# iamgroot42/A-LINK

Measured on AMD Instinct MI355X. Metric: 112x112 face embeddings/sec (IR-ResNet-100 ArcFace, 512-d, L2-normalised), higher is better.
Workload: dtype bf16

## Files before the change

a-link_amd/csrc/alink_common.h:

```cpp
#pragma once
#include <hip/hip_runtime.h>
#include <stdint.h>
#include <stddef.h>
#include <string>

#include "../../include/alink_hip.h"
#include "conv_kernel.h"

namespace alink {

void set_error(const char* fmt, ...);
int  hip_fail(hipError_t e, const char* what, const char* file, int line);

#define ALINK_HIP(call)                                                          \
    do {                                                                         \
        hipError_t e__ = (call);                                                 \
        if (e__ != hipSuccess) return ::alink::hip_fail(e__, #call, __FILE__, __LINE__); \
    } while (0)

#define ALINK_REQUIRE(cond, code, ...)          \
    do {                                        \
        if (!(cond)) {                          \
            ::alink::set_error(__VA_ARGS__);    \
            return (code);                      \
// ... 50 lines not shown
    int post_relu;
    int fine;
    int stagger;
    int ablate;
    float acc_scale;
    float bias_scale;
    float res_scale;
    int nprod;
    void* stamps;
};

hipError_t launch_conv_igemm(int dtype, const ConvParams& p, hipStream_t stream);
double     conv_flops(const ConvParams& p);

struct StemParams {
    const void*  in;
    const void*  wgt;
    const float* bias;
    const float* alpha;
    void*        out;
    int N, H, W, C0, layout;
    float sub[3], mul;
    int flip;
    float acc_scale, bias_scale;
};
hipError_t launch_stem(int dtype, const StemParams& p, hipStream_t stream);

struct FcFinishParams {
    const float* slabs;
    const float* bias;
    float*       out;
    float*       norms;
    int S, M, E;
    float scale;
    int*  nonfinite;
};
hipError_t launch_fc_finish(const FcFinishParams& p, hipStream_t stream);
hipError_t launch_absmax_f16(const void* x, size_t n_elements, unsigned* out_bits, hipStream_t stream);
hipError_t launch_conv_split_finish(int dtype, const ConvParams& p, const float* slabs, int S, hipStream_t stream);

ConvKernel direct_variant(int ksz, int stride, int pad, int H, int W, int Cin, int Cout);
ConvKernel direct_variant_tiles(int ksz, int stride, int pad, int H, int W, int Cin, int Cout);
ConvKernel linear_variant_x2(int ksz, int stride, int pad, int H, int W, int Cin, int Cout);
hipError_t launch_conv(ConvKernel k, int dtype, const ConvParams& p, hipStream_t st);
hipError_t direct_set_attributes();
ConvKernel linear_variant(int ksz, int stride, int pad, int H, int W, int Cin, int Cout);
ConvKernel c64_variant(int ksz, int stride, int pad, int H, int W, int Cin, int Cout);
ConvKernel s2c64_variant(int ksz, int stride, int pad, int H, int W, int Cin, int Cout);
hipError_t launch_conv3x3_linear(ConvKernel k, int dtype, const ConvParams& p, hipStream_t st);
hipError_t launch_conv3x3_c64(int dtype, const ConvParams& p, hipStream_t st);
hipError_t launch_conv3x3_s2c64(int dtype, const ConvParams& p, hipStream_t st);
hipError_t c64_set_attributes();
hipError_t s2c64_set_attributes();
hipError_t linear_set_attributes();
hipError_t linear_check_contract();
bool       front_c64_applies(int dtype, int H, int W, int C0, int Cout);
hipError_t front_c64_set_attributes();
hipError_t launch_front_c64(int dtype, const ConvParams& conv1, const StemParams& stem, void* xs, bool slopes_le_1, hipStream_t st);
bool       unit_c64_applies(int dtype, const ConvParams& c1, const ConvParams& c2);
hipError_t unit_c64_set_attributes();
hipError_t launch_unit_c64(int dtype, const ConvParams& c1, const ConvParams& c2, hipStream_t st);
bool       conv3x3_lat_applies(int dtype, const ConvParams& p);
hipError_t launch_conv3x3_lat(int dtype, const ConvParams& p, hipStream_t stream);
bool       conv_gemm_lat_applies(int dtype, const ConvParams& p);
hipError_t launch_conv_gemm_lat(int dtype, const ConvParams& p, hipStream_t stream);

hipError_t launch_l2norm_bwd(int dtype, const float* g, const float* e, const float* norms, void* dz, int M, int E,
                             hipStream_t st);
hipError_t launch_zero_insert(int dtype, const void* in, void* out, int N, int H, int W, int Ho, int Wo, int C,
                              hipStream_t st);
hipError_t launch_stem_bwd(int dtype, const void* dy0, const void* y0, const float* w, const float* alpha, float* dpix,
                           int N, int H, int W, float mul, int nchw, hipStream_t st);

hipError_t launch_r50_grad_scale(const float* dfeat, int count, int HW, float* scale, hipStream_t st);
hipError_t launch_r50_avgpool_bwd(int dtype, const float* dfeat, const void* y, void* dz, const float* scale, int N, int HW, int C,
                                  hipStream_t st);
hipError_t launch_r50_relu_mask(int dtype, void* g, const void* y, long long count, hipStream_t st);
hipError_t launch_r50_scatter_mask(int dtype, const void* in, const void* y, void* out, int N, int H, int W, int Ho, int Wo, int C,
                                   hipStream_t st);
hipError_t launch_r50_maxpool_bwd(int dtype, const void* y0, const void* pooled, const void* g, void* d0, int N, int H, int W, int C,
                                  int Hp, int Wp, hipStream_t st);
hipError_t launch_r50_stem_bwd(int dtype, const void* d0, const void* wfrag, float* dpix, const float* scale, int N, int H, int W,
                               int Ho, int Wo, int pad_t, int pad_l, int flip, hipStream_t st);
int r50_stem_bwd_max_width();

uint16_t f32_to_bf16_rne(float f);
uint16_t f32_to_f16_rne(float f);

int init_kernels();

__device__ __forceinline__ float relu_keep_nan(float v) { return v < 0.f ? 0.f : v; }
__device__ __forceinline__ float max_keep_nan(float a, float b) { return (a < b || b != b) ? b : a; }

}
#include <map>
#include <string>
#include <vector>
namespace alink {
struct F32Net;
F32Net* f32net_build(const std::map<std::string, std::vector<float>>& raw, const alink_ir_cfg& cfg);
void    f32net_destroy(F32Net* n);
size_t  f32net_workspace_bytes(const F32Net* n, int N);
int     f32net_embed(const F32Net* n, const void* dev_in, int layout, int N, float* dev_out, void* ws, size_t ws_bytes,
                     hipStream_t st);

}
```

a-link_amd/csrc/backbone.hip:

```cpp
#include "alink_common.h"

#include <algorithm>
#include <cmath>
#include <cstdarg>
#include <cstdio>
#include <cstring>
#include <map>
#include <string>
#include <vector>

namespace alink {

static thread_local char g_err[1024] = "";
void set_error(const char* fmt, ...) {
    va_list ap;
    va_start(ap, fmt);
    vsnprintf(g_err, sizeof(g_err), fmt, ap);
    va_end(ap);
}
int hip_fail(hipError_t e, const char* what, const char* file, int line) {
    set_error("HIP error %d (%s) in `%s` at %s:%d", (int)e, hipGetErrorString(e), what, file, line);
    return ALINK_EHIP;
}

// ... 642 lines not shown
        const bool wide = (L.Cout % 128) == 0;
        nwg = wide ? ((M + 127) / 128) * (L.Cout / 128) : ((M + 255) / 256) * (L.Cout / 64);
        units = L.ksz * L.ksz * ncc; kpu = 1;
    } else {
        return 1;
    }
    if (nwg > 64) return 1;
    int best = 1;
    for (int S = 2; S <= 8; ++S)
        if (units % S == 0 && units / S * kpu >= 4 && nwg * S <= 512 && (size_t)S * M * L.Cout * 4 <= SPLIT_SLAB_BYTES) best = S;
    return best;
}

int g_sibling_aware = 1;
extern "C" void alink_debug_set_sibling_aware(int on) { g_sibling_aware = on != 0; }
int g_fine_max = 384;
extern "C" void alink_debug_set_fine_max(int n) { g_fine_max = n; }
static int fine_form(ConvKernel k, long long M, int Cout, int siblings = 1) {
    if (!traits(k).fine) return 0;
    const int sib = (g_sibling_aware && k != ConvKernel::Linear7) ? siblings : 1;
    return linear_grid(M, Cout, 128) * sib <= g_fine_max ? 1 : 0;
}
int g_ablate = 0;
int g_stop_after = 0;
extern "C" void alink_debug_set_stop_after(int n) { g_stop_after = n; }
int g_stagger = 0;
int g_shard_stagger = 0;
extern "C" void alink_debug_set_shard_stagger(int on) { g_shard_stagger = on; }

int g_fuse_unit = 1;
constexpr int FUSE_UNIT_MIN_N = 64;
extern "C" void alink_debug_set_fuse_unit(int mode) { g_fuse_unit = mode; }
extern "C" void alink_debug_set_stagger(int n) { g_stagger = n < 0 ? 0 : n; }
void* g_stamps = nullptr;
int g_prof_reps = 4;
extern "C" void alink_debug_set_profile_reps(int n) { g_prof_reps = n < 1 ? 1 : n; }
extern "C" void alink_debug_set_ablate(int a) { g_ablate = a; }
extern "C" void alink_debug_set_stamps(void* p) { g_stamps = p; }

static const ConvLayer* fusable_unit(const alink_backbone* bb, const ConvLayer& L, int N, int S, bool cache) {
    if (!g_fuse_unit || (g_fuse_unit == 1 && N < FUSE_UNIT_MIN_N) || cache || S != 1 || g_ablate || g_stamps) return nullptr;
    const int dt = bb->cfg.dtype;
    if (dt != ALINK_DT_BF16 && dt != ALINK_DT_F16) return nullptr;
    const size_t i = (size_t)(&L - bb->convs.data());
    if (L.role != 1 || i + 1 >= bb->convs.size()) return nullptr;
    const ConvLayer& L2 = bb->convs[i + 1];
    if (L2.role != 3 || L2.unit != L.unit || L2.Cin2 || L2.in_buf != L.out_buf || L2.resid_buf != L.in_buf) return nullptr;
    if (L.kernel != ConvKernel::Linear56 || L2.kernel != ConvKernel::Linear56 || L.stride != 1 || L2.stride != 1) return nullptr;
    if (L.Cin != 64 || L.Cout != 64 || L2.Cin != 64 || L2.Cout != 64 || L.Hin != 56 || L.Win != 56) return nullptr;
    if (plan_split(bb, L2, N) != 1) return nullptr;
    return &L2;
}

static int embed_impl(alink_backbone_t* bb, const void* dev_in, int layout, int N, float* dev_out,
                      void* ws, size_t ws_bytes, hipStream_t stream, float* ms, double* flops, int* kind,
                      int* n_launches, const GradLayout* cache = nullptr, int calib = 0, hipEvent_t front_done = nullptr) {
    ALINK_REQUIRE(bb && dev_in && dev_out && ws, ALINK_EINVAL, "NULL argument");
    ALINK_REQUIRE(bb->finalized, ALINK_ESTATE, "alink_embed before alink_backbone_finalize");
    ALINK_REQUIRE(N > 0, ALINK_EINVAL, "n_images must be positive");
    ALINK_REQUIRE(layout >= 0 && layout <= 2, ALINK_EINVAL, "unknown pixel layout %d", layout);
    const alink_ir_cfg& cfg = bb->cfg;
    ALINK_REQUIRE((long long)N * cfg.height * cfg.width * 64 * (cfg.dtype == ALINK_DT_F16X2 ? 2 : 1) < (1ll << 31), ALINK_EINVAL,
                  "batch of %d images exceeds the 2^31-element activation limit; split the batch", N);
    size_t off[7], total;
    ws_layout(bb, N, off, &total);
    if (cache) total = cache->total;
    ALINK_REQUIRE(ws_bytes >= total, ALINK_ENOMEM, "workspace too small: %zu < %zu", ws_bytes, total);
    ALINK_REQUIRE(((uintptr_t)ws & 255) == 0, ALINK_EINVAL, "workspace must be 256-byte aligned");
    char* base = (char*)ws;
    auto buf = [&](int id) -> void* { return base + off[id]; };

    const bool prof = ms != nullptr;
    const int reps = prof ? g_prof_reps : 1;
    const int cap = prof ? *n_launches : 0;
    int nl = 0;
    std::vector<hipEvent_t> ev;
    std::vector<int> split_pairs;
    auto mark = [&]() -> int {
        if (!prof) return ALINK_OK;
        hipEvent_t e;
        ALINK_HIP(hipEventCreate(&e));
        ALINK_HIP(hipEventRecord(e, stream));
        ev.push_back(e);
        return ALINK_OK;
    };
    auto note = [&](double f, int k) {
        if (prof && nl < cap) { flops[nl] = f; kind[nl] = k; }
        ++nl;
    };
    int rc;
    if ((rc = mark())) return rc;

    const bool x2 = cfg.dtype == ALINK_DT_F16X2;
    ALINK_REQUIRE(!calib || x2, ALINK_ESTATE, "only the split-precision mode is calibrated");
    ALINK_REQUIRE(!x2 || calib || bb->calibrated, ALINK_ESTATE, "split-precision backbone: alink_backbone_calibrate has not run");
    int bexp[5] = {0, 0, 0, 0, 0};
    auto settle = [&](int* e_io, const void* out, size_t n_elems, auto&& launch) -> int {
        int e = *e_io;
        for (int attempt = 0; attempt < 24; ++attempt) {
            const int rcl = launch(e);
            if (rcl) return rcl;
            if (!calib) break;
            unsigned bits = 0;
            ALINK_HIP(hipMemsetAsync(bb->d_absmax, 0, 4, stream));
            ALINK_HIP(launch_absmax_f16(out, n_elems, bb->d_absmax, stream));
            ALINK_HIP(hipMemcpyAsync(&bits, bb->d_absmax, 4, hipMemcpyDeviceToHost, stream));
// ... 38 lines not shown
    }

    int last_out = 0, n_done = 0;
    bool front_marked = false;
    bool skip_conv2 = false;
    for (ConvLayer& L : bb->convs) {
        if (skip_conv2) { skip_conv2 = false; continue; }
        if (g_stop_after && n_done++ >= g_stop_after) return ALINK_OK;
        if (front_done && !front_marked && L.stage >= 1) {
            ALINK_HIP(hipEventRecord(front_done, stream));
            front_marked = true;
        }
        ConvParams p{};
        p.in = buf(L.in_buf); p.wgt = L.d_w; p.bias = L.d_bias; p.alpha = L.d_alpha;
        p.resid = L.resid_buf >= 0 ? buf(L.resid_buf) : nullptr;
        p.out = buf(L.out_buf); p.zero = bb->d_zero;
        if (cache) {
            if (L.role == 1) p.out = base + cache->toff[L.unit];
            if (L.role == 3) p.in = base + cache->toff[L.unit];
        }
        p.N = N; p.H = L.Hin; p.W = L.Win; p.Cin = L.Cin; p.Cout = L.Cout; p.Ho = L.Hout; p.Wo = L.Wout;
        p.stride = L.stride; p.ksz = L.ksz; p.pad = L.pad; p.M = N * L.Hout * L.Wout;
        p.border_cls = L.border_cls ? 1 : 0; p.splitk = 1;
        p.ksteps_per_split = L.ksz * L.ksz * (L.Cin / 64) + L.Cin2 / 64;
        if (L.Cin2) { p.in2 = buf(L.in2_buf); p.Cin2 = L.Cin2; p.in2_compact = (front && &L == &bb->convs[1]) ? 1 : 0; }
        p.ablate = g_ablate;
        p.stagger = g_stagger;
        p.nprod = (x2 && !calib) ? bb->products : 0;
        p.fine = fine_form(L.kernel, p.M, L.Cout, bb->siblings);
        int S = plan_split(bb, L, N);
        if (S > 1) {
            ConvParams probe = p;
            probe.splitk = 1;
            if (traits(L.kernel).split == SplitUnit::Chunk ? conv3x3_lat_applies(cfg.dtype, probe) : conv_gemm_lat_applies(cfg.dtype, probe)) S = 1;
        }
        if (x2) {
            p.ksteps_per_split *= 3;
            rc = settle(&L.e_out, p.out, (size_t)p.M * L.Cout * 2, [&](int e) -> int {
                p.acc_scale = std::ldexp(1.f, e - bexp[L.in_buf] - L.e_w);
                p.bias_scale = std::ldexp(1.f, e);
                p.res_scale = L.resid_buf >= 0 ? std::ldexp(1.f, e - bexp[L.resid_buf]) : 1.f;
                for (int r = 0; r < reps; ++r) {
                    ConvParams q = p;
                    if (S > 1) {
                        q.out = buf(6); q.splitk = S; q.ksteps_per_split = p.ksteps_per_split / S;
                    }
                    ALINK_HIP(launch_conv(L.kernel, cfg.dtype, q, stream));
                    if (S > 1) ALINK_HIP(launch_conv_split_finish(cfg.dtype, p, (const float*)buf(6), S, stream));
                }
                return ALINK_OK;
            });
            if (rc) return rc;
            bexp[L.out_buf] = L.e_out;
        } else if (front && &L == &bb->convs[0]) {
            p.stamps = g_stamps;
            for (int r = 0; r < reps; ++r) ALINK_HIP(launch_front_c64(cfg.dtype, p, sp, buf(0), bb->front_slopes_le_1, stream));
            note(conv_flops(p) + 2.0 * N * cfg.height * cfg.width * 64.0 * 27.0, 1);
            if ((rc = mark())) return rc;
            last_out = L.out_buf;
            continue;
        } else if (const ConvLayer* L2 = fusable_unit(bb, L, N, S, cache != nullptr)) {
            ConvParams p2 = p;
            p2.in = buf(L2->in_buf); p2.wgt = L2->d_w; p2.bias = L2->d_bias; p2.alpha = L2->d_alpha;
            p2.resid = buf(L2->resid_buf); p2.out = buf(L2->out_buf);
            p2.Cout = L2->Cout; p2.border_cls = L2->border_cls ? 1 : 0;
            ALINK_REQUIRE(unit_c64_applies(cfg.dtype, p, p2), ALINK_EINVAL, "fused unit %s: launch forms do not apply", L.name.c_str());
            for (int r = 0; r < reps; ++r) ALINK_HIP(launch_unit_c64(cfg.dtype, p, p2, stream));
            note(conv_flops(p), 1);
            if ((rc = mark())) return rc;
            if (prof && nl < cap) split_pairs.push_back(nl - 1);
            note(conv_flops(p2), 1);
            if ((rc = mark())) return rc;
            last_out = L2->out_buf;
            skip_conv2 = true;
            continue;
        } else
        for (int r = 0; r < reps; ++r) {
            ConvParams q = p;
            if (S > 1) {
                q.out = buf(6); q.splitk = S; q.ksteps_per_split = p.ksteps_per_split / S;
            }
            ALINK_HIP(launch_conv(L.kernel, cfg.dtype, q, stream));
            if (S > 1) ALINK_HIP(launch_conv_split_finish(cfg.dtype, p, (const float*)buf(6), S, stream));
        }
        note(conv_flops(p), 1);
        if ((rc = mark())) return rc;
        last_out = L.out_buf;
    }

    {
        ConvParams p{};
        p.in = buf(last_out); p.wgt = bb->d_fc_w; p.bias = nullptr; p.alpha = nullptr; p.resid = nullptr;
        p.out = buf(5); p.zero = bb->d_zero;
        p.N = N; p.H = 1; p.W = 1; p.Cin = bb->fc_K; p.Cout = cfg.emb; p.Ho = 1; p.Wo = 1;
        p.stride = 1; p.ksz = 1; p.pad = 0; p.M = N; p.border_cls = 0;
        p.splitk = bb->fc_splitk; p.ksteps_per_split = bb->fc_kps * (x2 ? 3 : 1);
        p.nprod = (x2 && !calib) ? bb->products : 0;
        ALINK_REQUIRE(p.splitk > 1, ALINK_EINVAL, "FC split-K must be > 1 (K=%d)", bb->fc_K);
        for (int r = 0; r < reps; ++r) ALINK_HIP(launch_conv_igemm(cfg.dtype, p, stream));
        note(conv_flops(p), 2);
        if ((rc = mark())) return rc;
        FcFinishParams f{};
        f.slabs = (const float*)buf(5); f.bias = bb->d_fc_bias; f.out = dev_out;
        f.norms = cache ? (float*)(base + cache->norms) : nullptr;
        f.S = bb->fc_splitk; f.M = N; f.E = cfg.emb;
        f.scale = x2 ? std::ldexp(1.f, -(bexp[last_out] + bb->fc_e_w)) : 1.f;
// ... 400 lines not shown
```

a-link_amd/csrc/conv3x3_direct.hip:

```cpp
#include "conv_device.h"

namespace alink {
namespace {

template <int WPX, int TPW, int TR>
struct Geo {
    static constexpr bool modeA = (TR % WPX) == 0;
    static constexpr bool modeB = !modeA && (TR == TPW);
    static constexpr bool modeC = !modeA && !modeB;
    static_assert(modeA || modeB || (TR == 1), "unsupported tile geometry");
    static constexpr int CPG = modeA ? TR / WPX : 1;
    static constexpr int R = modeA ? TPW / CPG : (modeB ? WPX : TPW * WPX);
    __device__ static constexpr int row(int g, int u) { return modeA ? u / CPG : (modeB ? g : g * TPW + u); }
    __device__ static constexpr int cb(int g, int u)  { return modeA ? g * CPG + u % CPG : (modeB ? u : 0); }
};

template <int A, int B>
struct IC2 { static constexpr int a = A, b = B; };

template <typename T, int WPX, int WCO, int TPW, int TCW, int TR, int PITCH, int NWB, int NWV, bool XDB>
__global__ __launch_bounds__(NWV * 64, 2) void conv3x3_direct_kernel(const ConvParams p) {
    typedef typename Vec8<T>::type vec8;
    typedef Geo<WPX, TPW, TR> G;
    constexpr int NT = NWV * 64;
// ... 257 lines not shown
typedef Variant<2, 4, 7, 2, 2, 32, 2>  D3;
typedef Variant<2, 4, 8, 2, 4, 64, 2>  D4;
typedef Variant<4, 2, 7, 2, 4, 64, 2>  D5;
typedef Variant<4, 2, 7, 2, 7, 128, 2> D6;
typedef Variant<2, 2, 7, 4, 1, 16, 2, 4, false> S1;
typedef Variant<2, 2, 7, 4, 2, 32, 2, 4, false> S3;

bool g_use_direct = true;
bool g_use_pair = true;

}

extern "C" void alink_debug_set_direct(int on) { g_use_direct = on != 0; }
extern "C" void alink_debug_set_pair(int on) { g_use_pair = on != 0; }

ConvKernel direct_variant(int ksz, int stride, int pad, int H, int W, int Cin, int Cout) {
    if (g_use_direct) {
        ConvKernel k = c64_variant(ksz, stride, pad, H, W, Cin, Cout);
        if (k == ConvKernel::Igemm) k = s2c64_variant(ksz, stride, pad, H, W, Cin, Cout);
        if (k != ConvKernel::Igemm) return k;
    }
    return direct_variant_tiles(ksz, stride, pad, H, W, Cin, Cout);
}
ConvKernel direct_variant_tiles(int ksz, int stride, int pad, int H, int W, int Cin, int Cout) {
    if (!g_use_direct || ksz != 3 || stride != 1 || pad != 1 || Cin % 64 || Cout % 64) return ConvKernel::Igemm;
    const ConvKernel lk = linear_variant(ksz, stride, pad, H, W, Cin, Cout);
    if (lk != ConvKernel::Igemm) return lk;
    if (W > 14 * 8 || H < 1) return ConvKernel::Igemm;
    const int tr = (W + 15) / 16, pitch = (W + 2 + 15) / 16 * 16;
    if (g_use_pair) {
        if (tr == 1 && pitch == 16 && W >= 12 && Cout % 128 == 0 && S1::lds_bytes(Cin) <= 80 * 1024) return ConvKernel::PairW14C128;
        if (tr == 2 && pitch == 32 && Cout % 128 == 0 && S3::lds_bytes(Cin) <= 80 * 1024) return ConvKernel::PairW28C128;
    }
    if (tr == 1 && pitch == 16 && W >= 12 && Cout % 256 == 0 && D1::fits(Cin)) return ConvKernel::TileW14C256;
    if (tr == 2 && pitch == 32 && Cout % 256 == 0 && D2::fits(Cin)) return ConvKernel::TileW28C256;
    if (tr == 2 && pitch == 32 && Cout % 128 == 0 && D3::fits(Cin)) return ConvKernel::TileW28C128;
    if (tr == 4 && pitch == 64 && Cout % 128 == 0 && D4::fits(Cin)) return ConvKernel::TileW56C128;
    if (tr == 4 && pitch == 64 && D5::fits(Cin)) return ConvKernel::TileW56C64;
    if (tr == 7 && pitch == 128 && W == 112 && D6::fits(Cin)) return ConvKernel::TileW112C64;
    return ConvKernel::Igemm;
}

hipError_t direct_set_attributes() {
    hipError_t e;
#define A(V)                                                         \
    if ((e = V::set_attr<__bf16>()) != hipSuccess) return e;         \
    if ((e = V::set_attr<_Float16>()) != hipSuccess) return e;
    A(D1) A(D2) A(D3) A(D4) A(D5) A(D6) A(S1) A(S3)
#undef A
    if ((e = c64_set_attributes()) != hipSuccess) return e;
    if ((e = front_c64_set_attributes()) != hipSuccess) return e;
    if ((e = s2c64_set_attributes()) != hipSuccess) return e;
    if ((e = unit_c64_set_attributes()) != hipSuccess) return e;
    return linear_set_attributes();
}

hipError_t launch_conv(ConvKernel k, int dtype, const ConvParams& p, hipStream_t st) {
    if (k == ConvKernel::Igemm) return launch_conv_igemm(dtype, p, st);
    if (k == ConvKernel::Roll112) return launch_conv3x3_c64(dtype, p, st);
    if (k == ConvKernel::Roll112S2) return launch_conv3x3_s2c64(dtype, p, st);
    if (traits(k).channel_block) return launch_conv3x3_linear(k, dtype, p, st);
    if (dtype != ALINK_DT_BF16 && dtype != ALINK_DT_F16) return hipErrorInvalidValue;
    if (p.ksz != 3 || p.stride != 1 || p.pad != 1 || p.splitk != 1) return hipErrorInvalidValue;
    if ((long long)p.N * p.H * p.W * p.Cin >= (1ll << 31)) return hipErrorInvalidValue;
#define L(V) (dtype == ALINK_DT_BF16 ? V::launch<__bf16>(p, st) : V::launch<_Float16>(p, st))
    switch (k) {
        case ConvKernel::TileW14C256: return L(D1);
        case ConvKernel::TileW28C256: return L(D2);
        case ConvKernel::TileW28C128: return L(D3);
        case ConvKernel::TileW56C128: return L(D4);
        case ConvKernel::TileW56C64:  return L(D5);
        case ConvKernel::TileW112C64: return L(D6);
        case ConvKernel::PairW14C128: return L(S1);
        case ConvKernel::PairW28C128: return L(S3);
        default: break;
    }
#undef L
    return hipErrorInvalidValue;
}

}
```

a-link_amd/csrc/conv3x3_s2c64.hip:

```cpp
#include "conv_device.h"

namespace alink {
namespace {

typedef __attribute__((__vector_size__(4 * sizeof(int)))) int i32x4;

constexpr int NT = 256;
constexpr int WI = 112, HI = 112, WO = 56, HO = 56, C = 64;
constexpr int RING = 8;
constexpr int ODDB = (WO + 8 + 1) * 128;
constexpr int EVENB = (WO + 8) * 128;
constexpr int PITCH = ODDB + EVENB;
constexpr int XBYTES = RING * PITCH;
constexpr int KR = 9 * C + C;
constexpr size_t lds_bytes() { return (size_t)XBYTES + C * 4; }

template <typename T, bool SC>
__global__ __launch_bounds__(NT, 1) void conv3x3_s2c64_kernel(const ConvParams p) {
    typedef typename Vec8<T>::type vec8;
    extern __shared__ __attribute__((aligned(16))) char smem[];

    const int tid = threadIdx.x, lane = tid & 63;
    const int wave = __builtin_amdgcn_readfirstlane(tid >> 6);
    const int th = wave >> 1, ch = wave & 1;
// ... 117 lines not shown
    auto top_of_pass = [&](bool staged, bool loaded, bool stored) __attribute__((always_inline)) {
        const int n = (staged ? 7 : 0) + (loaded ? 4 : 0) + (stored ? 2 : 0);
        switch (n) {
            case 13: wait_then_barrier<13>(); break;
            case 11: wait_then_barrier<11>(); break;
            case 9:  wait_then_barrier<9>(); break;
            case 7:  wait_then_barrier<7>(); break;
            case 6:  wait_then_barrier<6>(); break;
            case 4:  wait_then_barrier<4>(); break;
            case 2:  wait_then_barrier<2>(); break;
            default: wait_then_barrier<0>(); break;
        }
    };

    const long long nrows = (long long)p.N * HO;
    const long long r0 = nrows * blockIdx.x / gridDim.x, r1 = nrows * (blockIdx.x + 1) / gridDim.x;
    for (long long rr = r0; rr < r1;) {
        const long long n = rr / HO;
        const int y0 = (int)(rr - n * HO);
        int np = HO - y0;
        if (np > r1 - rr) np = (int)(r1 - rr);
        rr += np;
        const long long in_row0 = n * HI;
        wait_then_barrier<0>();
        stage_rows(in_row0, 2 * y0 - 1, 3);
        if (np > 1) stage_rows(in_row0, 2 * y0 + 2, 2);
        vec8 xsA[2][2], xsB[2][2];
        if (SC) load_sc(n, y0, xsA);
        f32x4 acc[2][2];
#pragma unroll 1
        for (int k = 0; k < np; k += 2) {
            if (k == 0) { if (np > 1) wait_then_barrier<7 + (SC ? 4 : 0)>(); else wait_then_barrier<SC ? 4 : 0>(); }
            else        top_of_pass(k + 1 < np, SC && k < np, true);
            if (k + 2 < np) stage_rows(in_row0, 2 * (y0 + k + 2), 2);
            if (SC && k + 1 < np) load_sc(n, y0 + k + 1, xsB);
            compute(acc, y0 + k, xsA);
            epilogue(acc, n, y0 + k);
            if (k + 1 < np) {
                top_of_pass(k + 2 < np, SC && k + 1 < np, true);
                if (k + 3 < np) stage_rows(in_row0, 2 * (y0 + k + 3), 2);
                if (SC && k + 2 < np) load_sc(n, y0 + k + 2, xsA);
                compute(acc, y0 + k + 1, xsB);
                epilogue(acc, n, y0 + k + 1);
            }
        }
    }
}

bool g_use_s2c64 = true;

}

extern "C" void alink_debug_set_s2direct(int on) { g_use_s2c64 = on != 0; }

ConvKernel s2c64_variant(int ksz, int stride, int pad, int H, int W, int Cin, int Cout) {
    if (!g_use_s2c64 || ksz != 3 || stride != 2 || pad != 1 || Cin != C || Cout != C || H != HI || W != WI) return ConvKernel::Igemm;
    return ConvKernel::Roll112S2;
}

hipError_t s2c64_set_attributes() {
    hipError_t e;
#define A(T, SC) if ((e = hipFuncSetAttribute((const void*)conv3x3_s2c64_kernel<T, SC>, hipFuncAttributeMaxDynamicSharedMemorySize, (int)lds_bytes())) != hipSuccess) return e;
    A(__bf16, true) A(__bf16, false) A(_Float16, true) A(_Float16, false)
#undef A
    return hipSuccess;
}

hipError_t launch_conv3x3_s2c64(int dtype, const ConvParams& p, hipStream_t st) {
    if (p.ksz != 3 || p.stride != 2 || p.pad != 1 || p.Cin != C || p.Cout != C || p.H != HI || p.W != WI) return hipErrorInvalidValue;
    if (p.splitk != 1 || p.dact || p.post_relu || p.border_cls || p.N <= 0) return hipErrorInvalidValue;
    if (p.in2 && (p.Cin2 != C || p.alpha || p.resid)) return hipErrorInvalidValue;
    if ((long long)p.N * HI * WI * C >= (1ll << 31)) return hipErrorInvalidValue;
    if (dtype != ALINK_DT_BF16 && dtype != ALINK_DT_F16) return hipErrorInvalidValue;
    const long long nrows = (long long)p.N * HO;
    const unsigned grid = (unsigned)(nrows < 256 ? nrows : 256);
    if (dtype == ALINK_DT_BF16) {
        if (p.in2) hipLaunchKernelGGL((conv3x3_s2c64_kernel<__bf16, true>), dim3(grid), dim3(NT), lds_bytes(), st, p);
        else       hipLaunchKernelGGL((conv3x3_s2c64_kernel<__bf16, false>), dim3(grid), dim3(NT), lds_bytes(), st, p);
    } else {
        if (p.in2) hipLaunchKernelGGL((conv3x3_s2c64_kernel<_Float16, true>), dim3(grid), dim3(NT), lds_bytes(), st, p);
        else       hipLaunchKernelGGL((conv3x3_s2c64_kernel<_Float16, false>), dim3(grid), dim3(NT), lds_bytes(), st, p);
    }
    return hipGetLastError();
}

}
```

include/alink_hip_debug.h:

```cpp
#ifndef ALINK_HIP_DEBUG_H
#define ALINK_HIP_DEBUG_H

#include <stddef.h>

#ifdef __cplusplus
extern "C" {
#endif

void alink_debug_set_linear(int mode);
void alink_debug_set_generic_epilogue(int on);
void alink_debug_set_direct(int on);
void alink_debug_set_pair(int on);
void alink_debug_set_c64(int on);
void alink_debug_set_s2direct(int on);
void alink_debug_set_fuse_stem(int on);
void alink_debug_set_fuse_unit(int mode);
void alink_debug_set_fuse_shortcut(int on);
void alink_debug_set_dma(int on);
void alink_debug_set_fine_max(int n);
void alink_debug_set_sibling_aware(int on);
void alink_debug_set_latency_form(int max_pixels);
void alink_debug_set_latency_tiles(int form);
void alink_debug_set_stagger(int n);
void alink_debug_set_shard_stagger(int on);

void alink_debug_set_tiny_step(int on);
void alink_debug_set_mini_step(int on);
void alink_debug_set_head_bf16_mfma(int on);

void alink_debug_set_smallres_overlap(int on);
void alink_debug_set_smallres_one_update(int on);

void alink_debug_set_stop_after(int n);
void alink_debug_set_profile_reps(int n);
void alink_debug_set_ablate(int a);
void alink_debug_set_stamps(void* dev_u64);
int alink_debug_lds_oob_probe(float* dev_out516, void* stream);
int alink_debug_linear_contract_ok(void);


struct alink_resnet50;
struct alink_backbone;
int alink_debug_resnet50_grad_cache_info(const struct alink_resnet50* r, int n_images, int index, size_t* byte_offset, int* H,
                                         int* W, int* C, char* name_buf, int name_len);
int alink_debug_backbone_grad_cache_info(const struct alink_backbone* bb, int n_images, int index, size_t* byte_offset, int* H,
                                         int* W, int* C, char* name_buf, int name_len);

#ifdef __cplusplus
}
#endif
#endif
```

Baseline: 47830.

## Fuse stem, first unit conv1 and stride-2 conv2 into one persistent kernel

Adds a new kernel that computes the stem 1x1 projection, the first unit's 3x3 conv1 with PReLU, and the stride-2 3x3 conv2 with its fused shortcut in a single launch. Rows stream through LDS ring buffers, and waves are specialised: four run conv1 while four run the stem and conv2. This removes the round trip of the 112x112x64 intermediate activations through global memory and one kernel launch. In exchange it needs a large LDS footprint and one block per CU with a grid capped at 256, which limits parallelism and adds pipeline fill overhead per block. It is enabled by default for batches of at least 64.

```diff
diff --git a/a-link_amd/csrc/alink_common.h b/a-link_amd/csrc/alink_common.h
--- a/a-link_amd/csrc/alink_common.h
+++ b/a-link_amd/csrc/alink_common.h
@@ -126,6 +126,7 @@
 hipError_t launch_conv3x3_s2c64(int dtype, const ConvParams& p, hipStream_t st);
 hipError_t c64_set_attributes();
 hipError_t s2c64_set_attributes();
+bool       s2c64_enabled();
 hipError_t linear_set_attributes();
 hipError_t linear_check_contract();
 bool       front_c64_applies(int dtype, int H, int W, int C0, int Cout);
@@ -134,6 +135,10 @@
 bool       unit_c64_applies(int dtype, const ConvParams& c1, const ConvParams& c2);
 hipError_t unit_c64_set_attributes();
 hipError_t launch_unit_c64(int dtype, const ConvParams& c1, const ConvParams& c2, hipStream_t st);
+bool       unit1_c64_applies(int dtype, const ConvParams& c1, const StemParams& stem, const ConvParams& c2);
+int        unit1_c64_mode();
+hipError_t unit1_c64_set_attributes();
+hipError_t launch_unit1_c64(int dtype, const ConvParams& c1, const StemParams& stem, const ConvParams& c2, bool slopes_le_1, hipStream_t st);
 bool       conv3x3_lat_applies(int dtype, const ConvParams& p);
 hipError_t launch_conv3x3_lat(int dtype, const ConvParams& p, hipStream_t stream);
 bool       conv_gemm_lat_applies(int dtype, const ConvParams& p);
diff --git a/a-link_amd/csrc/backbone.hip b/a-link_amd/csrc/backbone.hip
--- a/a-link_amd/csrc/backbone.hip
+++ b/a-link_amd/csrc/backbone.hip
@@ -718,6 +718,17 @@
     return &L2;
 }
 
+constexpr int FUSE_UNIT1_MIN_N = 64;
+static bool fusable_unit1(const alink_backbone* bb, bool front, int N, bool cache) {
+    const int mode = unit1_c64_mode();
+    if (!front || !mode || (mode == 1 && N < FUSE_UNIT1_MIN_N) || cache || g_ablate || g_stamps || !s2c64_enabled()) return false;
+    const ConvLayer& L = bb->convs[0];
+    const ConvLayer& L2 = bb->convs[1];
+    if (L.role != 1 || L2.role != 3 || L2.unit != L.unit || L2.in_buf != L.out_buf || L2.resid_buf >= 0) return false;
+    if (L2.kernel != ConvKernel::Roll112S2 || L2.Cin2 != 64 || L2.in2_buf != 0 || L2.Cout != 64) return false;
+    return plan_split(bb, L2, N) == 1;
+}
+
 static int embed_impl(alink_backbone_t* bb, const void* dev_in, int layout, int N, float* dev_out,
                       void* ws, size_t ws_bytes, hipStream_t stream, float* ms, double* flops, int* kind,
                       int* n_launches, const GradLayout* cache = nullptr, int calib = 0, hipEvent_t front_done = nullptr) {
@@ -862,6 +873,24 @@
             });
             if (rc) return rc;
             bexp[L.out_buf] = L.e_out;
+        } else if (front && &L == &bb->convs[0] && fusable_unit1(bb, front, N, cache != nullptr)) {
+            const ConvLayer& L2 = bb->convs[1];
+            ConvParams p2 = p;
+            p2.in = buf(L2.in_buf); p2.wgt = L2.d_w; p2.bias = L2.d_bias; p2.alpha = L2.d_alpha; p2.resid = nullptr;
+            p2.out = buf(L2.out_buf); p2.Cout = L2.Cout; p2.Ho = L2.Hout; p2.Wo = L2.Wout; p2.stride = L2.stride;
+            p2.M = N * L2.Hout * L2.Wout; p2.border_cls = L2.border_cls ? 1 : 0;
+            p2.in2 = buf(L2.in2_buf); p2.Cin2 = L2.Cin2; p2.in2_compact = 1;
+            p2.ksteps_per_split = L2.ksz * L2.ksz * (L2.Cin / 64) + L2.Cin2 / 64;
+            ALINK_REQUIRE(unit1_c64_applies(cfg.dtype, p, sp, p2), ALINK_EINVAL, "fused unit %s: launch forms do not apply", L.name.c_str());
+            for (int r = 0; r < reps; ++r) ALINK_HIP(launch_unit1_c64(cfg.dtype, p, sp, p2, bb->front_slopes_le_1, stream));
+            note(conv_flops(p) + 2.0 * N * cfg.height * cfg.width * 64.0 * 27.0, 1);
+            if ((rc = mark())) return rc;
+            if (prof && nl < cap) split_pairs.push_back(nl - 1);
+            note(conv_flops(p2), 1);
+            if ((rc = mark())) return rc;
+            last_out = L2.out_buf;
+            skip_conv2 = true;
+            continue;
         } else if (front && &L == &bb->convs[0]) {
             p.stamps = g_stamps;
             for (int r = 0; r < reps; ++r) ALINK_HIP(launch_front_c64(cfg.dtype, p, sp, buf(0), bb->front_slopes_le_1, stream));
diff --git a/a-link_amd/csrc/conv3x3_direct.hip b/a-link_amd/csrc/conv3x3_direct.hip
--- a/a-link_amd/csrc/conv3x3_direct.hip
+++ b/a-link_amd/csrc/conv3x3_direct.hip
@@ -333,6 +333,7 @@
     if ((e = front_c64_set_attributes()) != hipSuccess) return e;
     if ((e = s2c64_set_attributes()) != hipSuccess) return e;
     if ((e = unit_c64_set_attributes()) != hipSuccess) return e;
+    if ((e = unit1_c64_set_attributes()) != hipSuccess) return e;
     return linear_set_attributes();
 }
 
diff --git a/a-link_amd/csrc/conv3x3_s2c64.hip b/a-link_amd/csrc/conv3x3_s2c64.hip
--- a/a-link_amd/csrc/conv3x3_s2c64.hip
+++ b/a-link_amd/csrc/conv3x3_s2c64.hip
@@ -193,6 +193,7 @@
 }
 
 extern "C" void alink_debug_set_s2direct(int on) { g_use_s2c64 = on != 0; }
+bool s2c64_enabled() { return g_use_s2c64; }
 
 ConvKernel s2c64_variant(int ksz, int stride, int pad, int H, int W, int Cin, int Cout) {
     if (!g_use_s2c64 || ksz != 3 || stride != 2 || pad != 1 || Cin != C || Cout != C || H != HI || W != WI) return ConvKernel::Igemm;
diff --git a/a-link_amd/csrc/unit1_c64.hip b/a-link_amd/csrc/unit1_c64.hip
--- /dev/null
+++ b/a-link_amd/csrc/unit1_c64.hip
@@ -0,0 +1,418 @@
+#include "conv_device.h"
+
+namespace alink {
+namespace {
+
+typedef __attribute__((__vector_size__(4 * sizeof(int)))) int i32x4;
+typedef __attribute__((__vector_size__(2 * sizeof(int)))) int i32x2;
+
+__device__ __forceinline__ void lds_done_then_barrier() {
+    asm volatile("s_waitcnt lgkmcnt(0)\n\ts_barrier" ::: "memory");
+}
+
+template <int A>
+struct IC { static constexpr int a = A; };
+
+constexpr int NT = 512;
+constexpr int W = 112, H = 112, WO = 56, HO = 56;
+constexpr int SPITCH = (W + 2) * 128;
+constexpr int SR = 5;
+constexpr int ODDB = (WO + 1) * 128;
+constexpr int TPITCH = ODDB + WO * 128;
+constexpr int TR = 4;
+constexpr int IMPX = 32;
+constexpr int IMROWB = W * IMPX;
+constexpr int IR = 4;
+constexpr int TOFF = 0;
+constexpr int SOFF = TOFF + TR * TPITCH;
+constexpr int ZOFF = SOFF + SR * SPITCH;
+constexpr int IOFF = ZOFF + SPITCH;
+constexpr int BOFF = IOFF + IR * IMROWB;
+constexpr int TBYTES = 12 * 64 * 4;
+constexpr int SINKOFF = BOFF + TBYTES;
+constexpr size_t LDS_BYTES = (size_t)SINKOFF + 16;
+static_assert(LDS_BYTES <= 160 * 1024, "LDS budget");
+static_assert(ZOFF + ODDB + 64 * 128 <= (int)LDS_BYTES && SOFF + (SR - 1) * SPITCH + 128 * 128 <= (int)LDS_BYTES, "operand overrun stays inside LDS");
+
+struct Unit1Params {
+    const void*  w1;
+    const float* b1;
+    const float* a1;
+    const void*  w2;
+    const float* b2;
+    void*        out;
+    StemParams   s;
+    int N;
+};
+
+template <bool AMAX>
+__device__ __forceinline__ float prelu(float v, float slope) {
+    const float w = v * slope;
+    return AMAX ? __builtin_fmaxf(v, w) : (v > 0.f ? v : w);
+}
+
+template <typename T, bool AMAX, int HALF>
+__device__ __forceinline__ void conv1_wave(const Unit1Params& p, char* smem, int ch, int G0, int NP) {
+    typedef typename Vec8<T>::type vec8;
+    constexpr int NTL = HALF == 0 ? 4 : 3, U0 = HALF == 0 ? 0 : 4;
+    const int lane = threadIdx.x & 63, q = lane >> 4, lr = lane & 15;
+    const int d = delta(lr);
+
+    const T* __restrict__ gw = (const T*)p.w1;
+    vec8 wr[2][9][2];
+#pragma unroll
+    for (int ct = 0; ct < 2; ++ct)
+#pragma unroll
+        for (int tap = 0; tap < 9; ++tap)
+#pragma unroll
+            for (int ks = 0; ks < 2; ++ks)
+                wr[ct][tap][ks] = *(const vec8*)(gw + (size_t)(ch * 32 + 16 * ct + lr) * 576 + tap * 64 + ks * 32 + 8 * q);
+    int loff[3][2];
+#pragma unroll
+    for (int kx = 0; kx < 3; ++kx)
+#pragma unroll
+        for (int ks = 0; ks < 2; ++ks)
+            loff[kx][ks] = (d + kx) * 128 + ((((ks << 2) | q) ^ (((d + kx) >> 1) & 7)) << 4) + 2048 * U0;
+    const int tp0 = (d >> 1) + (d & 1);
+    const int tbase = ((d & 1) ? 0 : ODDB) + tp0 * 128;
+    const int jp = 4 * ch + q;
+    const float* const eb1 = (const float*)(smem + BOFF);
+    const float* const ea1 = eb1 + 9 * 64;
+
+#pragma unroll 1
+    for (int k = 0; k < NP; ++k) {
+        lds_done_then_barrier();
+        if (k < 6 || k > NP - 2) continue;
+        const int r = (G0 - 7 + k + H) % H;
+        int sb[3];
+#pragma unroll
+        for (int ky = 0; ky < 3; ++ky) sb[ky] = SOFF + ((k - 3 + ky) % SR) * SPITCH;
+        if (r == 0) sb[0] = ZOFF;
+        if (r == H - 1) sb[2] = ZOFF;
+
+        f32x4 acc[2][NTL];
+#pragma unroll
+        for (int ct = 0; ct < 2; ++ct)
+#pragma unroll
+            for (int u = 0; u < NTL; ++u) acc[ct][u] = f32x4{0.f, 0.f, 0.f, 0.f};
+        vec8 pf[2][NTL];
+#pragma unroll
+        for (int u = 0; u < NTL; ++u) pf[0][u] = *(const vec8*)(smem + (sb[0] + loff[0][0]) + 2048 * u);
+#pragma unroll
+        for (int st = 0; st < 18; ++st) {
+            if (st + 1 < 18) {
+                const int tn = (st + 1) >> 1, ksn = (st + 1) & 1;
+#pragma unroll
+                for (int u = 0; u < NTL; ++u)
+                    pf[(st + 1) & 1][u] = *(const vec8*)(smem + (sb[tn / 3] + loff[tn % 3][ksn]) + 2048 * u);
+            }
+            const int tap = st >> 1, ks = st & 1;
+#pragma unroll
+            for (int ct = 0; ct < 2; ++ct)
+#pragma unroll
+                for (int u = 0; u < NTL; ++u) acc[ct][u] = mfma16<T>(wr[ct][tap][ks], pf[st & 1][u], acc[ct][u]);
+        }
+
+        const int rc = r == 0 ? 0 : (r == H - 1 ? 2 : 1);
+        char* const tslot = smem + TOFF + (k & (TR - 1)) * TPITCH + tbase;
+        const f32x4 al0 = *(const f32x4*)(ea1 + ch * 32 + 8 * q), al1 = *(const f32x4*)(ea1 + ch * 32 + 8 * q + 4);
+#pragma unroll
+        for (int u = 0; u < NTL; ++u) {
+            const int x = 16 * (U0 + u) + d;
+            const int cls = rc * 3 + (x == 0 ? 0 : (x == W - 1 ? 2 : 1));
+            const f32x4 b0 = *(const f32x4*)(eb1 + cls * 64 + ch * 32 + 8 * q);
+            const f32x4 b1 = *(const f32x4*)(eb1 + cls * 64 + ch * 32 + 8 * q + 4);
+            float v[8];
+#pragma unroll
+            for (int j = 0; j < 4; ++j) { v[j] = acc[0][u][j] + b0[j]; v[4 + j] = acc[1][u][j] + b1[j]; }
+#pragma unroll
+            for (int i = 0; i < 8; ++i) v[i] = prelu<AMAX>(v[i], i < 4 ? al0[i & 3] : al1[i & 3]);
+            vec8 o8;
+#pragma unroll
+            for (int i = 0; i < 8; ++i) o8[i] = (T)v[i];
+            const int pos = 8 * (U0 + u) + tp0;
+            *(vec8*)(tslot + 1024 * (U0 + u) + ((jp ^ ((pos >> 1) & 7)) << 4)) = o8;
+        }
+    }
+}
+
+template <typename T, int LAYOUT, bool AMAX, int SHALF>
+__device__ __forceinline__ void stem_conv2_wave(const Unit1Params& p, char* smem, int b, int R0, int NP) {
+    typedef typename Vec8<T>::type vec8;
+    const StemParams& s = p.s;
+    const int tb = threadIdx.x - 256, lane = tb & 63, q = lane >> 4, lr = lane & 15;
+    const int d = delta(lr);
+    const int sch = b & 1;
+    const int cch = b >> 1, cct = b & 1;
+    const int G0 = 2 * R0;
+    const int last_row = p.N * H - 1;
+
+    vec8 swf[2][2];
+#pragma unroll
+    for (int t = 0; t < 2; ++t)
+#pragma unroll
+        for (int st = 0; st < 2; ++st) swf[t][st] = *(const vec8*)((const T*)s.wgt + (16 * (2 * sch + t) + lr) * 64 + st * 32 + 8 * q);
+    float sbi[8];
+#pragma unroll
+    for (int i = 0; i < 8; ++i) sbi[i] = s.bias[16 * q + 8 * sch + i];
+    const int rec_off = lr * IMPX + (q & 1) * 16;
+    const int sw_off = (lr + 1) * 128 + (((2 * q + sch) ^ (((lr + 1) >> 1) & 7)) << 4);
+
+    constexpr int KR = 9 * 64 + 64;
+    const T* __restrict__ gw2 = (const T*)p.w2 + (size_t)(cch * 32 + 16 * cct + lr) * KR + 8 * q;
+    vec8 w2r[9][2], ws[2];
+#pragma unroll
+    for (int tap = 0; tap < 9; ++tap)
+#pragma unroll
+        for (int ks = 0; ks < 2; ++ks) w2r[tap][ks] = *(const vec8*)(gw2 + tap * 64 + ks * 32);
+#pragma unroll
+    for (int ks = 0; ks < 2; ++ks) ws[ks] = *(const vec8*)(gw2 + 9 * 64 + ks * 32);
+    int loff2[2][2], scoff[2];
+#pragma unroll
+    for (int e = 0; e < 2; ++e)
+#pragma unroll
+        for (int ks = 0; ks < 2; ++ks) loff2[e][ks] = (d + e) * 128 + ((((ks << 2) | q) ^ (((d + e) >> 1) & 7)) << 4);
+#pragma unroll
+    for (int ks = 0; ks < 2; ++ks) scoff[ks] = (2 * d + 1) * 128 + ((((ks << 2) | q) ^ (d & 7)) << 4);
+    const float* const salpha = (const float*)(smem + BOFF) + 10 * 64;
+    const float* const eb2 = salpha + 64;
+
+    int goff[2], soff[2];
+    float ssub[2];
+    {
+        float sb0 = s.sub[0], sb1 = s.sub[1], sb2 = s.sub[2];
+        asm volatile("" : "+s"(sb0), "+s"(sb1), "+s"(sb2));
+#pragma unroll
+        for (int jj = 0; jj < 2; ++jj) {
+            const int i = tb + 256 * jj;
+            const bool valid = i < 3 * W;
+            const int e = valid ? i : 0;
+            int c, ix;
+            if (LAYOUT == ALINK_LAYOUT_NCHW_F32) { c = e / W; ix = e - c * W; }
+            else                                 { ix = e / 3; c = e - ix * 3; }
+            const int cn = s.flip ? 2 - c : c;
+            ssub[jj] = cn == 0 ? sb0 : (cn == 1 ? sb1 : sb2);
+            goff[jj] = LAYOUT == ALINK_LAYOUT_NCHW_F32 ? c * H * W + ix : e;
+            soff[jj] = valid ? (ix + 1) * IMPX + cn * 2 : -1;
+        }
+    }
+    constexpr int ROWP = LAYOUT == ALINK_LAYOUT_NCHW_F32 ? W : W * 3;
+    char* const sink = smem + SINKOFF;
+    auto load_row = [&](int g, float (&raw)[2]) __attribute__((always_inline)) {
+        g = g < 0 ? 0 : (g > last_row ? last_row : g);
+        const int n = g / H, iy = g - n * H;
+        const long long base = (long long)n * 3 * H * W + iy * ROWP;
+#pragma unroll
+        for (int jj = 0; jj < 2; ++jj) {
+            if (LAYOUT == ALINK_LAYOUT_NHWC_U8) raw[jj] = (float)((const uint8_t*)s.in)[base + goff[jj]];
+            else                                raw[jj] = ((const float*)s.in)[base + goff[jj]];
+        }
+    };
+    auto store_row = [&](int slot, const float (&raw)[2]) __attribute__((always_inline)) {
+        char* const rb = smem + IOFF + slot * IMROWB;
+#pragma unroll
+        for (int jj = 0; jj < 2; ++jj) {
+            const T v = (T)((raw[jj] - ssub[jj]) * s.mul);
+            char* const dst = rb + soff[jj];
+            *(T*)(soff[jj] >= 0 && soff[jj] < W * IMPX ? dst : sink) = v;
+            *(T*)(soff[jj] >= 0 ? dst - IMPX + 6 : sink) = v;
+            *(T*)(soff[jj] >= 2 * IMPX ? dst - 2 * IMPX + 12 : sink) = v;
+        }
+    };
+
+    float raw[2];
+    load_row(G0 - 3, raw);
+#pragma unroll 1
+    for (int k = 0; k < NP; ++k) {
+        lds_done_then_barrier();
+        store_row(k & (IR - 1), raw);
+        load_row(G0 - 2 + k, raw);
+
+        if (k >= 3 && k <= NP - 3) {
+            const int r = (G0 - 5 + k + H) % H;
+            const char* const rbm = smem + (r == 0 ? ZOFF : IOFF + ((k - 3) & (IR - 1)) * IMROWB);
+            const char* const rbz = smem + IOFF + ((k - 2) & (IR - 1)) * IMROWB;
+            const char* const rbp = smem + (r == H - 1 ? ZOFF : IOFF + ((k - 1) & (IR - 1)) * IMROWB);
+            const char* const wa = (q < 2 ? rbm : rbz) + rec_off;
+            const char* const wb = rbp + rec_off;
+            char* const ob = smem + SOFF + (k % SR) * SPITCH + sw_off;
+            const f32x4 sal0 = *(const f32x4*)(salpha + 16 * q + 8 * sch), sal1 = *(const f32x4*)(salpha + 16 * q + 8 * sch + 4);
+            auto group = [&](auto X0, auto NX) __attribute__((always_inline)) {
+                constexpr int x0 = decltype(X0)::a, nx = decltype(NX)::a;
+                vec8 pa[nx], pb[nx];
+#pragma unroll
+                for (int i = 0; i < nx; ++i) {
+                    pa[i] = *(const vec8*)(wa + 16 * IMPX * (x0 + i));
+                    pb[i] = *(const vec8*)(wb + 16 * IMPX * (x0 + i));
+                }
+                f32x4 a0[nx], a1[nx];
+#pragma unroll
+                for (int i = 0; i < nx; ++i) {
+                    a0[i] = mfma16<T>(swf[0][0], pa[i], f32x4{sbi[0], sbi[1], sbi[2], sbi[3]});
+                    a1[i] = mfma16<T>(swf[1][0], pa[i], f32x4{sbi[4], sbi[5], sbi[6], sbi[7]});
+                }
+#pragma unroll
+                for (int i = 0; i < nx; ++i) {
+                    a0[i] = mfma16<T>(swf[0][1], pb[i], a0[i]);
+                    a1[i] = mfma16<T>(swf[1][1], pb[i], a1[i]);
+                }
+#pragma unroll
+                for (int i = 0; i < nx; ++i) {
+                    vec8 o8;
+#pragma unroll
+                    for (int j = 0; j < 4; ++j) {
+                        o8[j] = (T)prelu<AMAX>(a0[i][j], sal0[j]);
+                        o8[4 + j] = (T)prelu<AMAX>(a1[i][j], sal1[j]);
+                    }
+                    *(vec8*)(ob + 2048 * (x0 + i)) = o8;
+                }
+            };
+            if (SHALF == 0) group(IC<0>{}, IC<4>{});
+            else            group(IC<4>{}, IC<3>{});
+        }
+
+        if ((k & 1) && k >= 9) {
+            const int Y = R0 + ((k - 9) >> 1);
+            const int y = Y % HO;
+            int sb[3];
+#pragma unroll
+            for (int ky = 0; ky < 3; ++ky) sb[ky] = TOFF + ((k - 3 + ky) & (TR - 1)) * TPITCH;
+            if (y == 0) sb[0] = ZOFF;
+            const int scb = SOFF + ((k - 4) % SR) * SPITCH;
+            f32x4 acc[4];
+#pragma unroll
+            for (int t = 0; t < 4; ++t) acc[t] = f32x4{0.f, 0.f, 0.f, 0.f};
+            auto frag = [&](int st, int t) __attribute__((always_inline)) -> vec8 {
+                const int tap = st >> 1, ks = st & 1, ky = tap / 3, kx = tap % 3;
+                return *(const vec8*)(smem + sb[ky] + loff2[kx == 2 ? 1 : 0][ks] + (kx == 1 ? ODDB : 0) + 2048 * t);
+            };
+            vec8 pf[2][4];
+#pragma unroll
+            for (int t = 0; t < 4; ++t) pf[0][t] = frag(0, t);
+            vec8 xs[2][4];
+#pragma unroll
+            for (int st = 0; st < 18; ++st) {
+                if (st + 1 < 18) {
+#pragma unroll
+                    for (int t = 0; t < 4; ++t) pf[(st + 1) & 1][t] = frag(st + 1, t);
+                } else {
+#pragma unroll
+                    for (int ks = 0; ks < 2; ++ks)
+#pragma unroll
+                        for (int t = 0; t < 4; ++t) xs[ks][t] = *(const vec8*)(smem + scb + scoff[ks] + 4096 * t);
+                }
+                const int tap = st >> 1, ks = st & 1;
+#pragma unroll
+                for (int t = 0; t < 4; ++t) acc[t] = mfma16<T>(w2r[tap][ks], pf[st & 1][t], acc[t]);
+            }
+#pragma unroll
+            for (int ks = 0; ks < 2; ++ks)
+#pragma unroll
+                for (int t = 0; t < 4; ++t) acc[t] = mfma16<T>(ws[ks], xs[ks][t], acc[t]);
+
+            const f32x4 b4 = *(const f32x4*)(eb2 + cch * 32 + 8 * q + 4 * cct);
+#pragma unroll
+            for (int t = 0; t < 4; ++t) {
+                const int x = 16 * t + d;
+                const bool live = x < WO;
+                const size_t el = ((size_t)Y * WO + (live ? x : 0)) * 64 + cch * 32 + 8 * q + 4 * cct;
+                vec8 o8;
+#pragma unroll
+                for (int j = 0; j < 4; ++j) { o8[j] = (T)(acc[t][j] + b4[j]); o8[4 + j] = (T)0.f; }
+                const i32x4 o4 = __builtin_bit_cast(i32x4, o8);
+                if (live) *(i32x2*)((T*)p.out + el) = i32x2{o4[0], o4[1]};
+            }
+        }
+    }
+}
+
+template <typename T, int LAYOUT, bool AMAX>
+__global__ __launch_bounds__(NT, 1) void unit1_c64_kernel(const Unit1Params p) {
+    extern __shared__ __attribute__((aligned(16))) char smem[];
+    const int tid = threadIdx.x;
+    for (int i = tid; i < TR * 8; i += NT) *(uint4*)(smem + TOFF + (i >> 3) * TPITCH + (i & 7) * 16) = uint4{0u, 0u, 0u, 0u};
+    for (int i = tid; i < SR * 16; i += NT) {
+        const int slot = i >> 4, side = (i >> 3) & 1, piece = i & 7;
+        *(uint4*)(smem + SOFF + slot * SPITCH + (side ? (W + 1) * 128 : 0) + piece * 16) = uint4{0u, 0u, 0u, 0u};
+    }
+    for (int i = tid; i < (SPITCH + IR * IMROWB) / 16; i += NT) *(uint4*)(smem + ZOFF + i * 16) = uint4{0u, 0u, 0u, 0u};
+    {
+        float* const tbl = (float*)(smem + BOFF);
+        for (int i = tid; i < 12 * 64; i += NT)
+            tbl[i] = i < 9 * 64 ? p.b1[i] : (i < 10 * 64 ? p.a1[i - 9 * 64] : (i < 11 * 64 ? p.s.alpha[i - 10 * 64] : p.b2[i - 11 * 64]));
+    }
+    const long long nrows = (long long)p.N * HO;
+    const int R0 = (int)(nrows * blockIdx.x / gridDim.x), R1 = (int)(nrows * (blockIdx.x + 1) / gridDim.x);
+    const int NP = 2 * (R1 - R0) + 8;
+    const int wave = __builtin_amdgcn_readfirstlane(tid >> 6);
+    if (wave < 4) {
+        if ((wave >> 1) == 0) conv1_wave<T, AMAX, 0>(p, smem, wave & 1, 2 * R0, NP);
+        else                  conv1_wave<T, AMAX, 1>(p, smem, wave & 1, 2 * R0, NP);
+    } else {
+        if (((wave - 4) >> 1) == 0) stem_conv2_wave<T, LAYOUT, AMAX, 1>(p, smem, wave - 4, R0, NP);
+        else                        stem_conv2_wave<T, LAYOUT, AMAX, 0>(p, smem, wave - 4, R0, NP);
+    }
+}
+
+int g_fuse_unit1 = 1;
+
+template <typename T, int LAYOUT>
+hipError_t unit1_attr() {
+    hipError_t e = hipFuncSetAttribute((const void*)unit1_c64_kernel<T, LAYOUT, true>, hipFuncAttributeMaxDynamicSharedMemorySize, (int)LDS_BYTES);
+    if (e != hipSuccess) return e;
+    return hipFuncSetAttribute((const void*)unit1_c64_kernel<T, LAYOUT, false>, hipFuncAttributeMaxDynamicSharedMemorySize, (int)LDS_BYTES);
+}
+
+template <typename T, int LAYOUT>
+void unit1_launch_l(const Unit1Params& p, bool amax, unsigned grid, hipStream_t st) {
+    if (amax) hipLaunchKernelGGL((unit1_c64_kernel<T, LAYOUT, true>), dim3(grid), dim3(NT), LDS_BYTES, st, p);
+    else      hipLaunchKernelGGL((unit1_c64_kernel<T, LAYOUT, false>), dim3(grid), dim3(NT), LDS_BYTES, st, p);
+}
+template <typename T>
+hipError_t unit1_launch(const Unit1Params& p, bool amax, unsigned grid, hipStream_t st) {
+    switch (p.s.layout) {
+        case ALINK_LAYOUT_NHWC_F32: unit1_launch_l<T, ALINK_LAYOUT_NHWC_F32>(p, amax, grid, st); break;
+        case ALINK_LAYOUT_NCHW_F32: unit1_launch_l<T, ALINK_LAYOUT_NCHW_F32>(p, amax, grid, st); break;
+        case ALINK_LAYOUT_NHWC_U8:  unit1_launch_l<T, ALINK_LAYOUT_NHWC_U8>(p, amax, grid, st); break;
+        default: return hipErrorInvalidValue;
+    }
+    return hipGetLastError();
+}
+
+}
+
+extern "C" void alink_debug_set_fuse_unit1(int mode) { g_fuse_unit1 = mode; }
+int unit1_c64_mode() { return g_fuse_unit1; }
+
+hipError_t unit1_c64_set_attributes() {
+    hipError_t e;
+    if ((e = unit1_attr<__bf16, ALINK_LAYOUT_NHWC_F32>()) != hipSuccess || (e = unit1_attr<__bf16, ALINK_LAYOUT_NCHW_F32>()) != hipSuccess ||
+        (e = unit1_attr<__bf16, ALINK_LAYOUT_NHWC_U8>()) != hipSuccess)
+        return e;
+    if ((e = unit1_attr<_Float16, ALINK_LAYOUT_NHWC_F32>()) != hipSuccess || (e = unit1_attr<_Float16, ALINK_LAYOUT_NCHW_F32>()) != hipSuccess ||
+        (e = unit1_attr<_Float16, ALINK_LAYOUT_NHWC_U8>()) != hipSuccess)
+        return e;
+    return hipSuccess;
+}
+
+bool unit1_c64_applies(int dtype, const ConvParams& c1, const StemParams& s, const ConvParams& c2) {
+    if (dtype != ALINK_DT_BF16 && dtype != ALINK_DT_F16) return false;
+    if (c1.ksz != 3 || c1.stride != 1 || c1.pad != 1 || c1.Cin != 64 || c1.Cout != 64 || c1.H != H || c1.W != W) return false;
+    if (s.H != H || s.W != W || s.C0 != 64 || s.N != c1.N || c1.N <= 0 || c2.N != c1.N) return false;
+    if (c1.splitk != 1 || c1.dact || c1.post_relu || c1.in2 || c1.resid || !c1.alpha || !c1.border_cls || c1.ablate || c1.stamps) return false;
+    if (c2.ksz != 3 || c2.stride != 2 || c2.pad != 1 || c2.Cin != 64 || c2.Cout != 64 || c2.H != H || c2.W != W) return false;
+    if (c2.splitk != 1 || c2.dact || c2.post_relu || c2.border_cls || !c2.in2 || c2.Cin2 != 64 || c2.alpha || c2.resid || c2.ablate || c2.stamps) return false;
+    return (long long)c1.N * H * W * 64 < (1ll << 31);
+}
+
+hipError_t launch_unit1_c64(int dtype, const ConvParams& c1, const StemParams& s, const ConvParams& c2, bool slopes_le_1, hipStream_t st) {
+    if (!unit1_c64_applies(dtype, c1, s, c2)) return hipErrorInvalidValue;
+    Unit1Params p{};
+    p.w1 = c1.wgt; p.b1 = c1.bias; p.a1 = c1.alpha; p.w2 = c2.wgt; p.b2 = c2.bias; p.out = c2.out; p.s = s; p.N = c1.N;
+    const long long nrows = (long long)p.N * HO;
+    const unsigned grid = (unsigned)(nrows < 256 ? nrows : 256);
+    if (dtype == ALINK_DT_BF16) return unit1_launch<__bf16>(p, slopes_le_1, grid, st);
+    return unit1_launch<_Float16>(p, slopes_le_1, grid, st);
+}
+
+}
diff --git a/include/alink_hip_debug.h b/include/alink_hip_debug.h
--- a/include/alink_hip_debug.h
+++ b/include/alink_hip_debug.h
@@ -15,6 +15,7 @@
 void alink_debug_set_s2direct(int on);
 void alink_debug_set_fuse_stem(int on);
 void alink_debug_set_fuse_unit(int mode);
+void alink_debug_set_fuse_unit1(int mode);
 void alink_debug_set_fuse_shortcut(int on);
 void alink_debug_set_dma(int on);
 void alink_debug_set_fine_max(int n);
```

Result: faster. 48590 (median of 6 runs) (+1.6%).
